# soedinglab/MMseqs2

Hardware: AMD Instinct MI355X
Metric: sw_gcells_per_s (higher is better)
Workload: dtype int16

## Files before the change

### mmseqs2_amd/csrc/pf_kernels.hip

```cpp
#include <type_traits>

#include "mmgpu_internal.h"
#include "pf_device.h"

namespace mmgpu {

namespace {

__device__ __forceinline__ PfCand *cand_slot(const PfDedupArgs &A, uint64_t bucket, uint32_t k) {
    return k < (uint32_t)PF_CAND0 ? A.cand_small + bucket * PF_CAND0 + k : A.cand + (A.cand_base[bucket] - A.cand_origin) + k;
}

struct __attribute__((packed, aligned(4))) U32Pair {
    uint32_t a, b;
};
struct __attribute__((packed, aligned(4))) U32Quad {
    uint32_t a, b, c, d;
};


constexpr uint32_t PF_COFS_KMERS = 12, PF_COFS_DWORDS = 4;

__global__ __launch_bounds__(256) void pf_cofs_kernel(const uint32_t *offsets, uint64_t table, uint32_t *cofs) {
    const uint64_t blk = (uint64_t)blockIdx.x * 256u + threadIdx.x;
// ... 536 lines not shown
    return o;
}
template <int NW>
__device__ __forceinline__ void load_cells(const uint8_t *p, uint32_t (&w)[NW]) {
    static_assert(NW == 4 || NW == 6, "16 or 24 bytes");
    const uintptr_t u = reinterpret_cast<uintptr_t>(p);
    const uint32_t *a = reinterpret_cast<const uint32_t *>(u & ~(uintptr_t)3);
    const uint32_t sh = (uint32_t)(u & 3u);
    const U32Quad d = *reinterpret_cast<const U32Quad *>(a);
    w[0] = __builtin_amdgcn_alignbyte(d.b, d.a, sh);
    w[1] = __builtin_amdgcn_alignbyte(d.c, d.b, sh);
    w[2] = __builtin_amdgcn_alignbyte(d.d, d.c, sh);
    if constexpr (NW == 4) {
        w[3] = __builtin_amdgcn_alignbyte(a[4], d.d, sh);
    } else {
        typedef uint32_t u32x3 __attribute__((ext_vector_type(3)));
        const u32x3 e = *reinterpret_cast<const u32x3 *>(a + 4);
        w[3] = __builtin_amdgcn_alignbyte(e.x, d.d, sh);
        w[4] = __builtin_amdgcn_alignbyte(e.y, e.x, sh);
        w[5] = __builtin_amdgcn_alignbyte(e.z, e.y, sh);
    }
}
template <int NW>
__device__ __forceinline__ Seg seg_cells_n(const uint32_t (&tw)[NW], const uint32_t (&qw)[NW], const uint32_t (&cw)[NW], int nn,
                                           const int8_t *smat) {
    Seg g;
    g.a = 0; g.b = 0; g.P = -(1 << 28); g.M = 0;
#pragma unroll
    for (int k = 0; k < 4 * NW; k++) {
        const uint32_t t5 = (tw[k >> 2] >> ((k & 3) * 8)) & 31u;
        const uint32_t q5 = (qw[k >> 2] >> ((k & 3) * 8)) & 31u;
        const int cb = (int)(int8_t)((cw[k >> 2] >> ((k & 3) * 8)) & 0xFFu);
        int x = (int)(int8_t)(smat[(q5 << 5) | t5] + cb);
        x = k < nn ? x : 0;
        g.b += x;
        g.a = max(0, g.a + x);
        g.P = max(g.P, g.b);
        g.M = max(g.M, g.a);
    }
    return g;
}
template <int NW>
__device__ __forceinline__ Seg seg_cells_rows_n(const uint32_t (&tw)[NW], const int8_t *rows, int nn) {
    Seg g;
    g.a = 0; g.b = 0; g.P = -(1 << 28); g.M = 0;
#pragma unroll
    for (int k = 0; k < 4 * NW; k++) {
        if (k < nn) {
            const int tb_ = (int)((tw[k >> 2] >> ((k & 3) * 8)) & 0xFFu);
            const int x = (int)rows[k * PF_PROW + (tb_ & (PF_PROW - 1))];
            g.b += x;
            g.a = max(0, g.a + x);
            g.P = max(g.P, g.b);
            g.M = max(g.M, g.a);
        }
    }
    return g;
}
__device__ __forceinline__ Seg seg_tree16(Seg g, int gl) {
#pragma unroll
    for (int d = 1; d < 16; d <<= 1) {
        Seg r;
        r.a = __shfl_down(g.a, d);
        r.b = __shfl_down(g.b, d);
        r.P = __shfl_down(g.P, d);
        r.M = __shfl_down(g.M, d);
        if ((gl & (2 * d - 1)) == 0) g = seg_combine(g, r);
    }
    return g;
}

template <bool SLOTS = true>
__device__ __forceinline__ uint64_t score_chunk(const PfDedupArgs &A, const int8_t *smat, uint64_t bucket, uint32_t q, uint32_t cb0,
                                                uint32_t nin, uint32_t ncand, PfCand c, int bshift, uint32_t *score_out = nullptr) {
    const int lane = lane_id();
    const int grp = lane >> 4, gl = lane & 15;
    const uint32_t qp0 = A.q_off[q];
    const int qlen = (int)(A.q_off[q + 1] - qp0);
    const uint8_t *qr = A.q_res + qp0;
    const uint8_t *qc = reinterpret_cast<const uint8_t *>(A.q_corr) + qp0;
    const bool has = (uint32_t)lane < nin;
    const int8_t *prows = (A.q_isprof && A.q_isprof[q]) ? A.q_rows + (size_t)qp0 * PF_PROW : nullptr;
    int my_len = 0, my_qs = 0;
    unsigned long long my_addr = 0;
    uint64_t cells = 0;
    if (has && !(A.q_nseg && A.q_nseg[q]))
        c.diag = (uint16_t)((c.diag & 0xFFu) | ((uint32_t)A.split_hi[(size_t)A.q_tile_base[q] * PF_T + c.score] << 8));
    if (has) {
        const int d = (int)(short)c.diag;
        const int tlen = (int)A.t_len[c.id];
        const uint8_t *t = A.t_res + (size_t)A.t_off4[c.id] * 4;
        const int mind = d < 0 ? -d : d;
        int ts = 0;
        if (d >= 0 && mind < qlen) {
            my_len = min(tlen, qlen - mind);
            my_qs = mind;
        } else if (d < 0 && mind < tlen) {
            my_len = min(tlen - mind, qlen);
            ts = mind;
        }
        my_addr = (unsigned long long)reinterpret_cast<uintptr_t>(t + ts);
        cells = (uint64_t)my_len;
        if (tlen >= 32768 && A.q_flags) atomicOr(&A.q_flags[q], 1u);
    }
    int my_score = 0;
    constexpr int UN = 2;
    auto trip = [&](auto nw_tag, const uint32_t k0) {
        constexpr int NW = decltype(nw_tag)::value;
        constexpr int CPL = 4 * NW, PASS = 16 * CPL;
        uint32_t tw[UN][NW], qw[UN][NW], cw[UN][NW];
        int len_u[UN], qs_u[UN];
        unsigned long long addr_u[UN];
#pragma unroll
        for (int u = 0; u < UN; u++) {
            const int src = (int)k0 + u * 4 + grp;
            len_u[u] = __shfl(my_len, src);
            qs_u[u] = __shfl(my_qs, src);
            addr_u[u] = __shfl(my_addr, src);
            if ((uint32_t)src >= nin) len_u[u] = 0;
#pragma unroll
            for (int z = 0; z < NW; z++) { tw[u][z] = 0; qw[u][z] = 0; cw[u][z] = 0; }
            if (gl * CPL < len_u[u]) {
                load_cells<NW>(reinterpret_cast<const uint8_t *>((uintptr_t)addr_u[u]) + gl * CPL, tw[u]);
                if (!prows) {
                    load_cells<NW>(qr + qs_u[u] + gl * CPL, qw[u]);
                    load_cells<NW>(qc + qs_u[u] + gl * CPL, cw[u]);
                }
            }
        }
#pragma unroll
        for (int u = 0; u < UN; u++) {
            const int len = len_u[u];
            Seg g;
            g.a = 0; g.b = 0; g.P = -(1 << 28); g.M = 0;
            if (gl * CPL < len) {
                if (prows) g = seg_cells_rows_n<NW>(tw[u], prows + (size_t)(qs_u[u] + gl * CPL) * PF_PROW, min(CPL, len - gl * CPL));
                else g = seg_cells_n<NW>(tw[u], qw[u], cw[u], min(CPL, len - gl * CPL), smat);
            }
            g = seg_tree16(g, gl);
            int sc = 0, best = 0;
            if (gl == 0 && len > 0) {
                best = max(g.M, g.P);
                sc = max(g.a, g.b);
            }
            int maxlen = len;
            maxlen = max(maxlen, __shfl_xor(maxlen, 16));
            maxlen = max(maxlen, __shfl_xor(maxlen, 32));
            for (int p0 = PASS; p0 < maxlen; p0 += PASS) {
                const int o = p0 + gl * CPL;
                Seg h;
                h.a = 0; h.b = 0; h.P = -(1 << 28); h.M = 0;
                if (o < len) {
                    uint32_t t2[NW], q2[NW], c2[NW];
                    load_cells<NW>(reinterpret_cast<const uint8_t *>((uintptr_t)addr_u[u]) + o, t2);
                    if (prows) h = seg_cells_rows_n<NW>(t2, prows + (size_t)(qs_u[u] + o) * PF_PROW, min(CPL, len - o));
                    else {
                        load_cells<NW>(qr + qs_u[u] + o, q2);
                        load_cells<NW>(qc + qs_u[u] + o, c2);
                        h = seg_cells_n<NW>(t2, q2, c2, min(CPL, len - o), smat);
                    }
                }
                h = seg_tree16(h, gl);
                if (gl == 0 && p0 < len) {
                    best = max(best, max(h.M, sc + h.P));
                    sc = max(h.a, sc + h.b);
                }
            }
            const int r0 = __shfl(best, 0), r1 = __shfl(best, 16), r2 = __shfl(best, 32), r3 = __shfl(best, 48);
            const int rel = lane - ((int)k0 + u * 4);
            if (rel >= 0 && rel < 4) my_score = rel == 0 ? r0 : (rel == 1 ? r1 : (rel == 2 ? r2 : r3));
        }
    };
    for (uint32_t k0 = 0; k0 < nin; k0 += 4 * UN) {
        const bool mine = (uint32_t)lane >= k0 && (uint32_t)lane < k0 + 4u * UN && has;
        if (ballot(mine && my_len > 256)) trip(std::integral_constant<int, 6>{}, k0);
        else trip(std::integral_constant<int, 4>{}, k0);
    }
    c.score = (uint32_t)my_score;
    if (score_out) *score_out = c.score;
    if constexpr (!SLOTS) return cells;
    if (has) {
        PfCand *slot = cand_slot(A, bucket, cb0 + (uint32_t)lane);
// ... 26 lines not shown
    return cells;
}

constexpr int REPLAY_WAVES_PER_EU = 4;
constexpr int REPLAY_PD = 4;


struct ReplayLds {
    uint32_t prev[4][PF_IDS_PER_BIN / 4];
    uint32_t last[4][PF_IDS_PER_BIN / 4];
    uint32_t emit[4][PF_IDS_PER_BIN / 32];
    uint32_t cand[4][3][64];
    uint8_t mark[4][64];
    int8_t smat[32 * 32];
};

__device__ __forceinline__ uint32_t lds_byte_exchange(uint32_t *word, uint32_t shift, uint32_t byte) {
    uint32_t old;
    const uint32_t addr = (uint32_t)(uintptr_t)word;
    asm volatile("ds_mskor_rtn_b32 %0, %1, %2, %3\n\ts_waitcnt lgkmcnt(0)" : "=v"(old) : "v"(addr), "v"(0xFFu << shift), "v"(byte << shift) : "memory");
    return old;
}

template <bool SEGS>
__device__ __forceinline__ void replay_bucket_impl(const PfDedupArgs &A, ReplayLds &M, uint64_t bucket) {
    const int lane = lane_id(), wave = (int)(threadIdx.x >> 6);
    const uint32_t B = A.bins;
    const uint32_t q = (uint32_t)(bucket / B), bin = (uint32_t)(bucket % B);
    const uint32_t ntiles = A.q_ntiles[q];
    if (ntiles == 0) {
        if (lane == 0) A.cand_count[bucket] = 0;
        return;
    }
    const uint32_t tb = A.q_tile_base[q];
    uint32_t *P = M.prev[wave];
    uint32_t *L = M.last[wave];
    uint32_t *E = M.emit[wave];
    uint8_t *mark = M.mark[wave];
    const int bshift = pf_bin_shift(B);
    auto clear_state = [&]() {
        uint4 *P4 = reinterpret_cast<uint4 *>(P);
        for (int k = lane; k < PF_IDS_PER_BIN / 16; k += 64) P4[k] = make_uint4(0u, 0u, 0u, 0u);
        for (int k = lane; k < PF_IDS_PER_BIN / 32; k += 64) E[k] = 0;
    };
    clear_state();

    uint32_t ncand = 0;
// ... 90 lines not shown
        request(64u, e1, tile1, at1);
        request(128u, e2, tile2, at2);
        request(192u, e3, tile3, at3);
        for (uint32_t xg = 0; xg < total; xg += 64u * REPLAY_PD) {
            one_round(xg, e0, tile0, at0);
            one_round(xg + 64u, e1, tile1, at1);
            one_round(xg + 128u, e2, tile2, at2);
            one_round(xg + 192u, e3, tile3, at3);
        }
    }
    if (lane == 0) {
        A.cand_count[bucket] = ncand;
        if (!SEGS && ncand > 64 && A.big_list) A.big_list[atomicAdd(A.big_count, 1u)] = (uint32_t)(bucket - (uint64_t)A.q_first * B);
    }
    if (!SEGS && ncand > 0 && ncand <= 64) {
        PfCand c = pf_cand_zero();
        if ((uint32_t)lane < ncand) {
            const uint32_t kd = M.cand[wave][0][lane];
            c.id = ((kd & 0xFFFu) << bshift) | bin;
            c.arr = M.cand[wave][1][lane];
            c.diag = (uint16_t)(kd >> 12);
            c.score = M.cand[wave][2][lane];
        }
        uint64_t cells = score_chunk(A, M.smat, bucket, q, 0, ncand, ncand, c, bshift);
        if (A.cell_counter) wave_sum_to((unsigned long long *)&A.cell_counter[q], cells);
    }
}

__global__ __launch_bounds__(256) __attribute__((amdgpu_waves_per_eu(REPLAY_WAVES_PER_EU))) void pf_replay_kernel(PfDedupArgs A) {
    __shared__ ReplayLds M;
    pf_load_smat32<256>(M.smat, A.mat, A.alphabet);
    __syncthreads();
    uint64_t bucket;
    if (!pf_wave_bucket(A, 4u, &bucket)) return;
    if (A.q_nseg && A.q_nseg[(uint32_t)(bucket / A.bins)]) replay_bucket_impl<true>(A, M, bucket);
    else replay_bucket_impl<false>(A, M, bucket);
}

__device__ __forceinline__ void ungapped_bucket(const PfDedupArgs &A, const int8_t *smat, uint64_t bucket) {
    const int lane = lane_id();
    const uint32_t B = A.bins;
    const uint32_t ncand = A.cand_count[bucket];
    const uint32_t q = (uint32_t)(bucket / B);
    if (ncand <= 64 || (A.q_nseg && A.q_nseg[q])) return;
    const int bshift = pf_bin_shift(B);
    uint64_t cells = 0;
    for (uint32_t cb0 = 0; cb0 < ncand; cb0 += 64) {
        const uint32_t nin = min(64u, ncand - cb0);
        PfCand c = pf_cand_zero();
        if ((uint32_t)lane < nin) c = *cand_slot(A, bucket, cb0 + (uint32_t)lane);
        cells += score_chunk(A, smat, bucket, q, cb0, nin, ncand, c, bshift);
    }
    if (A.cell_counter) wave_sum_to((unsigned long long *)&A.cell_counter[q], cells);
}

__global__ __launch_bounds__(256) void pf_ungapped_kernel(PfDedupArgs A) {
    __shared__ int8_t smat[32 * 32];
    const int wave = (int)(threadIdx.x >> 6);
    pf_load_smat32<256>(smat, A.mat, A.alphabet);
    __syncthreads();
    const uint32_t B = A.bins;
    if (A.big_list) {
        const uint32_t n = *A.big_count;
        for (uint32_t i = blockIdx.x * 4u + (uint32_t)wave; i < n; i += gridDim.x * 4u) ungapped_bucket(A, smat, (uint64_t)A.q_first * B + A.big_list[i]);
        return;
    }
    const uint64_t bucket = (uint64_t)A.q_first * B + (uint64_t)blockIdx.x * 4u + (uint32_t)wave;
    if (bucket >= (uint64_t)(A.q_first + A.n_queries) * B) return;
    ungapped_bucket(A, smat, bucket);
}

__global__ __launch_bounds__(256) void pf_count_kernel(PfDedupArgs A) {
    __shared__ uint16_t s_state[4][PF_IDS_PER_BIN];
    __shared__ uint32_t s_emit[4][PF_IDS_PER_BIN / 32];
    const int lane = lane_id(), wave = (int)(threadIdx.x >> 6);
    const uint32_t B = A.bins;
    uint64_t bucket;
    if (!pf_wave_bucket(A, 4u, &bucket)) return;
    const uint32_t q = (uint32_t)(bucket / B), bin = (uint32_t)(bucket % B);
    const uint32_t ntiles = A.q_ntiles[q];
    if (lane == 0) A.cand_count[bucket] = 0;
    if (ntiles == 0) return;
    const uint32_t tb = A.q_tile_base[q];
    uint16_t *S = s_state[wave];
    uint32_t *E = s_emit[wave];
    const int bshift = pf_bin_shift(B);
    for (int k = lane; k < PF_IDS_PER_BIN; k += 64) S[k] = 0;
    for (int k = lane; k < PF_IDS_PER_BIN / 32; k += 64) E[k] = 0;
    uint32_t ncand = 0;
    const uint64_t below = lanes_below(lane);
    for (uint32_t t0 = 0; t0 < ntiles; t0 += 64) {
        const uint32_t tl = t0 + (uint32_t)lane;
// ... 127 lines not shown
            const PfCand *cp = cand_slot(A, bucket, ci);
            atomicMax(&S[cp->id >> bshift], keepmax_key(min(255u, cp->score), ci));
        }
        __syncthreads();
        PfCand *surv = A.surv + (A.cand_base[(uint64_t)q * B] - A.cand_origin);
        for (uint32_t c0 = 0; c0 < ncand; c0 += 1024) {
            const uint32_t ci = c0 + threadIdx.x;
            bool win = false;
            PfCand c = pf_cand_zero();
            if (ci < ncand) {
                c = *cand_slot(A, bucket, ci);
                const uint32_t cnt = min(255u, c.score);
                win = S[c.id >> bshift] == keepmax_key(cnt, ci) && cnt >= A.min_diag_score;
            }
            wave_append(&A.surv_count[q], surv, win, c);
        }
        __syncthreads();
    }
}

constexpr int PF_LONG_POOL = 4096;
constexpr uint32_t PF_LONG_NONE = 0xFFFFu;

__device__ int wave_diag_score(const int8_t *smat, const uint8_t *qr, const uint8_t *qc, const int8_t *prows, int qlen, const uint8_t *t,
                               int tlen, int diag) {
    const int lane = lane_id();
    const int mind = diag < 0 ? -diag : diag;
    int len, qs, ts;
    if (diag >= 0 && mind < qlen) {
        len = min(tlen, qlen - mind);
        qs = mind;
        ts = 0;
    } else if (diag < 0 && mind < tlen) {
        len = min(tlen - mind, qlen);
        qs = 0;
        ts = mind;
    } else {
        return 0;
    }
    int sc = 0, best = 0;
    for (int p0 = 0; p0 < len; p0 += 1024) {
        const int o = p0 + lane * 16;
        Seg h;
        h.a = 0; h.b = 0; h.P = -(1 << 28); h.M = 0;
        if (o < len) {
            uint32_t tw[4], qw[4], cw[4];
            load_cells<4>(t + ts + o, tw);
            if (prows) h = seg_cells_rows_n<4>(tw, prows + (size_t)(qs + o) * PF_PROW, min(16, len - o));
            else {
                load_cells<4>(qr + qs + o, qw);
                load_cells<4>(qc + qs + o, cw);
                h = seg_cells_n<4>(tw, qw, cw, min(16, len - o), smat);
            }
        }
        h = seg_tree16(h, lane & 15);
        Seg g[4];
#pragma unroll
        for (int k = 0; k < 4; k++) {
            g[k].a = __shfl(h.a, 16 * k);
            g[k].b = __shfl(h.b, 16 * k);
            g[k].P = __shfl(h.P, 16 * k);
            g[k].M = __shfl(h.M, 16 * k);
        }
        const Seg all = seg_combine(seg_combine(g[0], g[1]), seg_combine(g[2], g[3]));
        best = max(best, max(all.M, sc + all.P));
        sc = max(all.a, sc + all.b);
    }
    return best;
}

__device__ int wave_long_score(const int8_t *smat, const uint8_t *qr, const uint8_t *qc, const int8_t *prows, int qlen, const uint8_t *t,
                               int tlen, uint32_t diag16) {
    int total = 0;
    for (uint32_t d = 1; d <= 1u + (uint32_t)tlen / 32768u; d++)
        total = max(total, wave_diag_score(smat, qr, qc, prows, qlen, t, tlen, (int)(0u - d * 65536u + diag16)));
    for (uint32_t d = 0; d <= (uint32_t)qlen / 65536u; d++)
        total = max(total, wave_diag_score(smat, qr, qc, prows, qlen, t, tlen, (int)(d * 65536u + diag16)));
    return total;
}

__global__ __launch_bounds__(256) void pf_longq_kernel(PfDedupArgs A) {
    __shared__ int8_t smat[32 * 32];
    const int lane = lane_id();
    pf_load_smat32<256>(smat, A.mat, A.alphabet);
    __syncthreads();
    const uint32_t B = A.bins;
    uint64_t bucket;
    if (!pf_wave_bucket(A, 4u, &bucket)) return;
    const uint32_t q = (uint32_t)(bucket / B);
    const uint32_t qp0 = A.q_off[q];
    const int qlen = (int)(A.q_off[q + 1] - qp0);
    if (qlen < 32768) return;
    if (lane == 0 && bucket == (uint64_t)q * B) atomicOr(&A.q_flags[q], 1u);
    if (A.nucl || (A.q_nseg && A.q_nseg[q])) return;
    const uint8_t *qr = A.q_res + qp0;
    const uint8_t *qc = reinterpret_cast<const uint8_t *>(A.q_corr) + qp0;
    const int8_t *prows = (A.q_isprof && A.q_isprof[q]) ? A.q_rows + (size_t)qp0 * PF_PROW : nullptr;
    const uint32_t ncand = A.cand_count[bucket];
    for (uint32_t ci = 0; ci < ncand; ci++) {
        PfCand *slot = cand_slot(A, bucket, ci);
        const uint32_t id = slot->id;
        const int own = wave_long_score(smat, qr, qc, prows, qlen, A.t_res + (size_t)A.t_off4[id] * 4, (int)A.t_len[id], slot->diag);
        if (lane == 0) slot->score = (uint32_t)own;
    }
}

__global__ __launch_bounds__(256) void pf_long_kernel(PfDedupArgs A) {
    __shared__ uint32_t s_tab[PF_IDS_PER_BIN];
    __shared__ uint32_t s_dbits[65536 / 32];
    __shared__ uint64_t s_key[PF_LONG_POOL];
    __shared__ uint32_t s_ci[PF_LONG_POOL];
    __shared__ uint16_t s_bucket[PF_LONG_POOL];
    __shared__ uint16_t s_job[PF_LONG_POOL];
    __shared__ int8_t smat[32 * 32];
    __shared__ uint32_t sh_npool, sh_nlong;
    const uint32_t q = A.q_first + blockIdx.x;
    if (!(A.q_flags[q] & 1u)) return;
    if (A.nucl || (A.q_nseg && A.q_nseg[q])) return;
    const int lane = lane_id(), wave = (int)(threadIdx.x >> 6);
    const uint32_t B = A.bins;
    const int bshift = pf_bin_shift(B);
    pf_load_smat32<256>(smat, A.mat, A.alphabet);
    for (int k = (int)threadIdx.x; k < 65536 / 32; k += 256) s_dbits[k] = 0;
    if (threadIdx.x == 0) {
        sh_npool = 0;
// ... 50 lines not shown
            uint32_t lo = p, hi = p;
            while (lo > 0 && (s_key[lo - 1] >> 43) == d) lo--;
            while (hi + 1 < npool && (s_key[hi + 1] >> 43) == d) hi++;
            const uint32_t r = p - lo, n_d = hi - lo + 1, b0 = (r / 8u) * 8u;
            if (b0 + 8u > n_d) job = (uint16_t)p;
            else {
                uint32_t h = 0;
                for (uint32_t z = lo + b0; z < p; z++) h += s_ci[z] >> 31;
                const uint32_t e = lo + b0 + h;
                job = (s_ci[e] >> 31) ? (uint16_t)e : (uint16_t)PF_LONG_NONE;
            }
            atomicAdd(&sh_nlong, 1u);
        }
        s_job[p] = job;
    }
    __syncthreads();
    const uint8_t *qr = A.q_res + qp0;
    const uint8_t *qc = reinterpret_cast<const uint8_t *>(A.q_corr) + qp0;
    const int8_t *prows = (A.q_isprof && A.q_isprof[q]) ? A.q_rows + (size_t)qp0 * PF_PROW : nullptr;
    for (uint32_t p = (uint32_t)wave; p < npool; p += 4) {
        if (!(s_ci[p] >> 31)) continue;
        PfCand *slot = cand_slot(A, (uint64_t)q * B + s_bucket[p], s_ci[p] & 0x7FFFFFFFu);
        const uint32_t id = slot->id, d16 = slot->diag;
        const int own = wave_long_score(smat, qr, qc, prows, qlen, A.t_res + (size_t)A.t_off4[id] * 4, (int)A.t_len[id], d16);
        int by = 0;
        const uint32_t job = s_job[p];
        if (job == p) by = own;
        else if (job != PF_LONG_NONE) {
            const uint32_t id2 = cand_slot(A, (uint64_t)q * B + s_bucket[job], s_ci[job] & 0x7FFFFFFFu)->id;
            by = wave_long_score(smat, qr, qc, prows, qlen, A.t_res + (size_t)A.t_off4[id2] * 4, (int)A.t_len[id2], d16);
        }
        const uint32_t cnt = (uint32_t)min(255, by), ex = (uint32_t)own;
        if (lane == 0) slot->score = (cnt == min(255u, ex)) ? ex : (0x80000000u | (cnt << 23) | (ex & 0x7FFFFFu));
    }
    }
    __threadfence();
    __syncthreads();
    if (threadIdx.x == 0) A.surv_count[q] = 0;
    __syncthreads();
    PfCand *surv = A.surv + (A.cand_base[(uint64_t)q * B] - A.cand_origin);
    for (uint32_t bk = 0; bk < B; bk++) {
        const uint64_t bucket = (uint64_t)q * B + bk;
        const uint32_t ncand = A.cand_count[bucket];
        if (ncand == 0) continue;
        for (uint32_t ci = threadIdx.x; ci < ncand; ci += 256) s_tab[cand_slot(A, bucket, ci)->id >> bshift] = 0;
        __syncthreads();
        for (uint32_t ci = threadIdx.x; ci < ncand; ci += 256) {
            const PfCand *cp = cand_slot(A, bucket, ci);
            atomicMax(&s_tab[cp->id >> bshift], keepmax_key(pf_el_count(cp->score), ci));
        }
        __syncthreads();
        for (uint32_t ci = threadIdx.x; ci < ncand; ci += 256) {
            const PfCand c = *cand_slot(A, bucket, ci);
// ... 105 lines not shown
        if (nseg >= (uint32_t)PF_MAX_SEG) { nseg = PF_MAX_SEG + 1; break; }
        nseg++;
        if (lane == 0) seg[nseg] = start;
        seg_begin = start;
        lcur = lo;
    }
    if (lane == 0) {
        A.q_nseg[q] = nseg;
        A.q_final[q] = total - seg_begin;
    }
}

__device__ __forceinline__ PfOvfElem ovf_from_cand(const PfCand &c, uint32_t step) {
    PfOvfElem e;
    e.id = c.id;
    e.score = 0;
    e.ord = ((long long)step << 33) + (long long)c.arr;
    e.diag = c.diag;
    e.pad0 = 0;
    e.pad1 = 0;
    return e;
}

__global__ __launch_bounds__(256) void pf_overflow_kernel(PfOvfArgs A) {
    __shared__ uint32_t s_tab[4][PF_IDS_PER_BIN];
    __shared__ int8_t smat[32 * 32];
    const PfDedupArgs &D = A.D;
    const int lane = lane_id(), wave = (int)(threadIdx.x >> 6);
    pf_load_smat32<256>(smat, D.mat, D.alphabet);
    __syncthreads();
    const uint32_t B = D.bins;
    const uint64_t w = (uint64_t)blockIdx.x * 4u + (uint32_t)wave;
    if (w >= (uint64_t)A.n_ovf * B) return;
    const uint32_t qi = (uint32_t)(w / B), bin = (uint32_t)(w % B);
    const uint32_t q = A.ovf_queries[qi];
    const uint32_t ns = D.q_nseg[q];
    const uint32_t step = A.step;
    if (ns > (uint32_t)PF_MAX_SEG || step > ns + 1) return;
    const bool final_step = step == ns + 1;
    if (final_step && A.q_final[q] == 0) return;
    const uint64_t bucket = (uint64_t)q * B + bin;
    const uint32_t ncand = D.cand_count[bucket];
    uint32_t *tab = s_tab[wave];
    const int bshift = pf_bin_shift(B);
    const uint64_t below = lanes_below(lane);
    const uint64_t base = A.ovf_base[qi] + (uint64_t)(D.cand_base[bucket] - D.cand_base[(uint64_t)q * B]);
// ... 93 lines not shown
        if (lane == 0) {
            A.o_count[(size_t)qi * B + bin] = n;
            if (n) atomicAdd(&totals[step], n);
        }
        return;
    }
    for (uint32_t r0 = 0; r0 < n; r0 += 64) {
        const uint32_t idx = r0 + (uint32_t)lane;
        const bool need = idx < n && cur[idx].score == 0;
        const uint64_t nb = ballot(need);
        if (!nb) continue;
        const uint32_t cnt = (uint32_t)__popcll(nb), mine = (uint32_t)__popcll(nb & below);
        if (need) tab[mine] = (uint32_t)lane;
        __builtin_amdgcn_wave_barrier();
        const int src = (uint32_t)lane < cnt ? (int)tab[lane] : 0;
        const uint32_t my_id = idx < n ? cur[idx].id : 0u, my_diag = idx < n ? (uint32_t)cur[idx].diag : 0u;
        PfCand c;
        c.id = (uint32_t)__shfl((int)my_id, src);
        c.arr = 0;
        c.score = 0;
        c.diag = (uint16_t)__shfl((int)my_diag, src);
        c.pad = 0;
        uint32_t sc = 0;
        (void)score_chunk<false>(D, smat, bucket, q, 0, cnt, 65u, c, bshift, &sc);
        tab[64 + lane] = sc;
        __builtin_amdgcn_wave_barrier();
        if (need) cur[idx].score = tab[64 + mine];
    }
    __threadfence();
    for (int k = lane; k < PF_IDS_PER_BIN; k += 64) tab[k] = 0;
    for (uint32_t r0 = 0; r0 < n; r0 += 64) {
        const uint32_t idx = r0 + (uint32_t)lane;
        if (idx < n) {
            const uint32_t cnt = min(255u, cur[idx].score);
            atomicMax(&tab[cur[idx].id >> bshift], keepmax_key(cnt, idx));
        }
    }
    PfOvfElem *dst = cur == O ? S : O;
    uint32_t m = 0;
    PfCand *surv = D.surv + (D.cand_base[(uint64_t)q * B] - D.cand_origin);
    for (uint32_t r0 = 0; r0 < n; r0 += 64) {
        const uint32_t idx = r0 + (uint32_t)lane;
        bool keep = false;
        PfOvfElem e;
        e.id = 0; e.score = 0; e.ord = 0; e.diag = 0; e.pad0 = 0; e.pad1 = 0;
        if (idx < n) {
            e = cur[idx];
// ... 37 lines not shown
            if (m) atomicAdd(&totals[step], m);
        }
    }
}

__device__ uint32_t list_ordinal(const PfSelectArgs &A, uint32_t q, uint32_t arr) {
    const uint32_t p0 = A.q_off[q], p1 = A.q_off[q + 1];
    uint32_t lo = p0, hi = p1 - 1;
    while (lo < hi) {
        const uint32_t mid = (lo + hi + 1) >> 1;
        if (A.peb[mid] <= arr) lo = mid; else hi = mid - 1;
    }
    const uint32_t rel = arr - A.peb[lo];
    uint32_t a = A.list_base[lo], b = A.list_base[lo + 1];
    if (b <= a) return a - A.list_base[p0];
    b -= 1;
    while (a < b) {
        const uint32_t mid = (a + b + 1) >> 1;
        if (A.lists[mid].lprefix <= rel) a = mid; else b = mid - 1;
    }
    return a - A.list_base[p0];
}

template <bool XCHG, bool BIG>
__global__ __launch_bounds__(256) void pf_select_kernel(PfSelectArgs A) {
    __shared__ uint32_t hist[256];
    __shared__ uint32_t sh_thr, sh_trunc, sh_nelig, sh_nsel, sh_ntie;
    __shared__ uint64_t sh_prefix, sh_mask;
    __shared__ uint32_t sh_remaining;
    __shared__ uint64_t skey_lds[BIG ? 1 : PF_MAX_HITS];
    __shared__ uint16_t sdiag_lds[BIG ? 1 : PF_MAX_HITS];
    const uint32_t q = A.q_first + blockIdx.x;
    uint64_t *skey = BIG ? A.big_keys + (size_t)q * A.big_stride : skey_lds;
    uint16_t *sdiag = BIG ? A.big_diags + (size_t)q * A.big_stride : sdiag_lds;
    const uint32_t sort_cap = BIG ? A.big_stride : (uint32_t)PF_MAX_HITS;
    const uint32_t n = A.surv_count[q];
    const PfCand *S = A.surv + (A.cand_base[(uint64_t)q * A.bins] - A.cand_origin);
    const uint32_t ident = A.q_identity[q];
    const uint32_t max_hits = A.max_hits;
    mmgpu_pf_hit *out = A.hits + (size_t)q * A.hit_stride;

    for (int k = (int)threadIdx.x; k < 256; k += 256) hist[k] = 0;
    if (threadIdx.x == 0) sh_remaining = 0;
    __syncthreads();
    if (A.cand_count != nullptr) {
        uint32_t loc = 0;
        for (uint32_t k = threadIdx.x; k < A.bins; k += 256) loc += A.cand_count[(uint64_t)q * A.bins + k];
        for (int d = 1; d < 64; d <<= 1) loc += __shfl_xor(loc, d);
        if ((threadIdx.x & 63u) == 0 && loc) atomicAdd(&sh_remaining, loc);
        __syncthreads();
        if (threadIdx.x == 0 && sh_remaining >= A.cand_cap && A.q_flags) A.q_flags[q] |= 2u;
        __syncthreads();
    }
    for (uint32_t k = threadIdx.x; k < n; k += 256) atomicAdd(&hist[pf_el_count(S[k].score)], 1u);
    __syncthreads();
    if (threadIdx.x == 0) {
        const uint32_t dthr = pf_score_threshold(hist, max_hits, A.min_diag_score);
        sh_thr = dthr;
        sh_trunc = (dthr >= 255u && !A.kmer_score) ? 1u : 0u;
        sh_nelig = 0;
        sh_nsel = 0;
    }
    __syncthreads();
    const uint32_t dthr = sh_thr;
    const bool trunc = sh_trunc != 0;
    const int ms = pf_self_clamp(A.q_self_score[q]);
    const float fms = (float)ms;
    const uint32_t refmask = A.ref_bins - 1;

    auto key_of = [&](const PfCand &c, bool *elig) -> uint64_t {
        const uint32_t cnt = pf_el_count(c.score);
        uint32_t kc;
        if (trunc) {
            *elig = cnt >= 255u && c.id != ident;
            kc = rescaled_count(pf_el_exact(c.score), fms);
        } else {
            *elig = cnt >= dthr && c.id != ident;
            kc = cnt;
        }
        const uint64_t ord = (A.nucl && cnt >= 255u) ? (uint64_t)c.id : (((uint64_t)c.pad << 32) | (uint64_t)c.arr);
        const uint32_t gid = XCHG ? A.global_ids[c.id] : c.id;
        if (XCHG) *elig = trunc ? cnt >= 255u : cnt >= dthr;
        return ((uint64_t)(255u - kc) << 56) | ((uint64_t)(gid & refmask) << 45) | (ord & ((1ull << 45) - 1));
    };

    uint32_t mine = 0;
    for (uint32_t k = threadIdx.x; k < n; k += 256) {
        bool el;
        (void)key_of(S[k], &el);
        mine += el ? 1u : 0u;
    }
    if (mine) atomicAdd(&sh_nelig, mine);
    __syncthreads();
    const uint32_t nelig = sh_nelig;
    const uint32_t has_ident = (!XCHG && ident != 0xFFFFFFFFu) ? 1u : 0u;
    const uint32_t want = max_hits > has_ident ? max_hits - has_ident : 0u;

    uint64_t kstar = ~0ull;
    if (nelig > want && want > 0) {
        if (threadIdx.x == 0) {
            sh_prefix = 0;
            sh_mask = 0;
            sh_remaining = want;
        }
        __syncthreads();
        for (int shift = 56; shift >= 0; shift -= 8) {
            for (int k = (int)threadIdx.x; k < 256; k += 256) hist[k] = 0;
            __syncthreads();
            const uint64_t prefix = sh_prefix, mask = sh_mask;
            for (uint32_t k = threadIdx.x; k < n; k += 256) {
                bool el;
                const uint64_t key = key_of(S[k], &el);
                if (el && (key & mask) == prefix) atomicAdd(&hist[(uint32_t)(key >> shift) & 0xFFu], 1u);
            }
            __syncthreads();
            if (threadIdx.x == 0) {
                uint32_t rem = sh_remaining, cum = 0, d = 0;
                for (d = 0; d < 256; d++) {
                    if (cum + hist[d] >= rem) break;
                    cum += hist[d];
                }
                sh_remaining = rem - cum;
                sh_prefix = prefix | ((uint64_t)d << shift);
                sh_mask = mask | (0xFFull << shift);
                sh_ntie = hist[d];
            }
            __syncthreads();
            if (!BIG && shift == 56 && sh_ntie <= sort_cap) {
                const uint32_t m = sh_ntie, rem = sh_remaining;
                const uint64_t prefix1 = sh_prefix;
                __syncthreads();
                if (threadIdx.x == 0) sh_ntie = 0;
                __syncthreads();
                for (uint32_t k = threadIdx.x; k < n; k += 256) {
                    bool el;
                    const uint64_t key = key_of(S[k], &el);
                    if (el && (key & (0xFFull << 56)) == prefix1) skey[atomicAdd(&sh_ntie, 1u)] = key;
                }
                uint32_t mp2 = 1;
                while (mp2 < m) mp2 <<= 1;
                __syncthreads();
                for (uint32_t k = m + threadIdx.x; k < mp2; k += 256) skey[k] = ~0ull;
                __syncthreads();
                block_bitonic_sort<256>(mp2, [&](uint32_t i, uint32_t j) { return skey[i] > skey[j]; }, [&](uint32_t i, uint32_t j) { exchange_at(skey, i, j); });
                if (threadIdx.x == 0) sh_prefix = skey[rem - 1];
                __syncthreads();
                break;
            }
        }
        kstar = sh_prefix;
// ... 170 lines not shown
    const uint64_t words = (table + 31) / 32;
    hipLaunchKernelGGL(pf_bitmap_kernel, dim3((unsigned)((words + 255) / 256)), dim3(256), 0, s, offsets, table, bitmap, nonempty);
    return hipGetLastError();
}

hipError_t launch_pf_scan(const uint32_t *in, const uint32_t *q_off, uint32_t nq, const uint64_t *base, uint32_t *out,
                          uint64_t *totals, hipStream_t s) {
    if (nq == 0) return hipSuccess;
    hipLaunchKernelGGL(pf_scan_kernel, dim3(nq), dim3(256), 0, s, in, q_off, nq, base, out, totals);
    return hipGetLastError();
}

hipError_t launch_pf_split(const PfSplitArgs &A, uint32_t n_tiles, hipStream_t s) {
    if (n_tiles == 0) return hipSuccess;
    hipLaunchKernelGGL(pf_split_kernel, dim3(n_tiles), dim3(SPW * 64), (size_t)SPW * A.bins * sizeof(uint16_t), s, A);
    return hipGetLastError();
}

hipError_t launch_pf_dedup(const PfDedupArgs &A, hipEvent_t after_replay, hipEvent_t after_ungapped, hipStream_t s) {
    const uint64_t buckets = (uint64_t)A.n_queries * A.bins;
    if (buckets == 0) return hipSuccess;
    const dim3 grid((unsigned)((buckets + 3) / 4)), block(256);
    hipError_t e;
    hipLaunchKernelGGL(pf_replay_kernel, grid, block, 0, s, A);
    if ((e = hipGetLastError()) != hipSuccess) return e;
    if (after_replay && (e = hipEventRecord(after_replay, s)) != hipSuccess) return e;
    const dim3 grid_big(A.big_list ? (unsigned)std::min<uint64_t>((buckets + 3) / 4, 2048) : grid.x);
    hipLaunchKernelGGL(pf_ungapped_kernel, grid_big, block, 0, s, A);
    if ((e = hipGetLastError()) != hipSuccess) return e;
    if (after_ungapped && (e = hipEventRecord(after_ungapped, s)) != hipSuccess) return e;
    if (A.nucl) hipLaunchKernelGGL(pf_keepmax_nucl_kernel, dim3((unsigned)((buckets + 1) / 2)), dim3(128), 0, s, A);
    else if (A.big_list) hipLaunchKernelGGL(pf_keepmax_list_kernel, dim3((unsigned)std::min<uint64_t>(buckets, 1024)), dim3(1024), 0, s, A);
    else hipLaunchKernelGGL(pf_keepmax_kernel, grid, block, 0, s, A);
    return hipGetLastError();
}

hipError_t launch_pf_long(const PfDedupArgs &A, bool long_queries, hipStream_t s) {
    if (A.n_queries == 0 || A.q_flags == nullptr) return hipSuccess;
    if (long_queries) {
        const uint64_t buckets = (uint64_t)A.n_queries * A.bins;
        hipLaunchKernelGGL(pf_longq_kernel, dim3((unsigned)((buckets + 3) / 4)), dim3(256), 0, s, A);
        if (hipError_t e = hipGetLastError(); e != hipSuccess) return e;
    }
    hipLaunchKernelGGL(pf_long_kernel, dim3(A.n_queries), dim3(256), 0, s, A);
    return hipGetLastError();
}

hipError_t launch_pf_count(const PfDedupArgs &A, hipEvent_t after_a, hipEvent_t after_b, hipStream_t s) {
    const uint64_t buckets = (uint64_t)A.n_queries * A.bins;
    if (buckets == 0) return hipSuccess;
    hipLaunchKernelGGL(pf_count_kernel, dim3((unsigned)((buckets + 3) / 4)), dim3(256), 0, s, A);
    hipError_t e = hipGetLastError();
    if (e != hipSuccess) return e;
    if (after_a && (e = hipEventRecord(after_a, s)) != hipSuccess) return e;
    if (after_b && (e = hipEventRecord(after_b, s)) != hipSuccess) return e;
    return hipSuccess;
}

hipError_t launch_pf_segments(const PfSegArgs &A, hipStream_t s) {
    if (A.n_ovf == 0) return hipSuccess;
    hipLaunchKernelGGL(pf_segments_kernel, dim3(A.n_ovf), dim3(64), 0, s, A);
    return hipGetLastError();
}

hipError_t launch_pf_overflow(const PfOvfArgs &A, hipStream_t s) {
    const uint64_t waves = (uint64_t)A.n_ovf * A.D.bins;
    if (waves == 0) return hipSuccess;
    hipLaunchKernelGGL(pf_overflow_kernel, dim3((unsigned)((waves + 3) / 4)), dim3(256), 0, s, A);
    return hipGetLastError();
}

hipError_t launch_pf_merge(const PfMergeArgs &A, hipStream_t s) {
    if (A.nq == 0) return hipSuccess;
    hipLaunchKernelGGL(pf_merge_kernel, dim3(A.nq), dim3(256), 0, s, A);
    return hipGetLastError();
}

hipError_t launch_pf_select(const PfSelectArgs &A, uint32_t nq, hipStream_t s) {
    if (nq == 0) return hipSuccess;
    if (A.xhits) hipLaunchKernelGGL((pf_select_kernel<true, false>), dim3(nq), dim3(256), 0, s, A);
    else if (A.big_keys) hipLaunchKernelGGL((pf_select_kernel<false, true>), dim3(nq), dim3(256), 0, s, A);
    else hipLaunchKernelGGL((pf_select_kernel<false, false>), dim3(nq), dim3(256), 0, s, A);
    return hipGetLastError();
}

void warm_pf() {
    hipFuncAttributes a;
    (void)hipFuncGetAttributes(&a, reinterpret_cast<const void *>(&pf_kmers_kernel<true>));
}

}
```

Measured before the change: 4899.

## Branch-free ungapped cells, DPP tree reduction, histogram-based eligibility and smaller select LDS

```diff
diff --git a/mmseqs2_amd/csrc/pf_kernels.hip b/mmseqs2_amd/csrc/pf_kernels.hip
--- a/mmseqs2_amd/csrc/pf_kernels.hip
+++ b/mmseqs2_amd/csrc/pf_kernels.hip
@@ -582,8 +582,8 @@
     }
 }
 template <int NW>
-__device__ __forceinline__ Seg seg_cells_n(const uint32_t (&tw)[NW], const uint32_t (&qw)[NW], const uint32_t (&cw)[NW], int nn,
-                                           const int8_t *smat) {
+__device__ __forceinline__ Seg seg_cells_select_n(const uint32_t (&tw)[NW], const uint32_t (&qw)[NW], const uint32_t (&cw)[NW], int nn,
+                                                  const int8_t *smat) {
     Seg g;
     g.a = 0; g.b = 0; g.P = -(1 << 28); g.M = 0;
 #pragma unroll
@@ -601,6 +601,37 @@
     return g;
 }
 template <int NW>
+__device__ __forceinline__ Seg seg_cells_n(const uint32_t (&tw)[NW], const uint32_t (&qw_in)[NW], const uint32_t (&cw_in)[NW], int nn,
+                                           const int8_t *smat, bool zrow) {
+    if (!zrow) return seg_cells_select_n<NW>(tw, qw_in, cw_in, nn, smat);
+    uint32_t qw[NW], cw[NW];
+#pragma unroll
+    for (int z = 0; z < NW; z++) { qw[z] = qw_in[z]; cw[z] = cw_in[z]; }
+    if (nn < 4 * NW) {
+#pragma unroll
+        for (int z = 0; z < NW; z++) {
+            const int bits = min(32, max(0, 8 * nn - 32 * z));
+            const uint32_t kill = (uint32_t)(0xFFFFFFFFull << bits);
+            qw[z] = (qw[z] & ~kill) | (0x1F1F1F1Fu & kill);
+            cw[z] &= ~kill;
+        }
+    }
+    Seg g;
+    g.a = 0; g.b = 0; g.P = -(1 << 28); g.M = 0;
+#pragma unroll
+    for (int k = 0; k < 4 * NW; k++) {
+        const uint32_t t5 = (tw[k >> 2] >> ((k & 3) * 8)) & 31u;
+        const uint32_t q5 = (qw[k >> 2] >> ((k & 3) * 8)) & 31u;
+        const int cb = (int)(int8_t)((cw[k >> 2] >> ((k & 3) * 8)) & 0xFFu);
+        const int x = (int)(int8_t)(smat[(q5 << 5) | t5] + cb);
+        g.b += x;
+        g.a = max(0, g.a + x);
+        g.P = max(g.P, g.b);
+        g.M = max(g.M, g.a);
+    }
+    return g;
+}
+template <int NW>
 __device__ __forceinline__ Seg seg_cells_rows_n(const uint32_t (&tw)[NW], const int8_t *rows, int nn) {
     Seg g;
     g.a = 0; g.b = 0; g.P = -(1 << 28); g.M = 0;
@@ -617,29 +648,38 @@
     }
     return g;
 }
+template <int D>
+__device__ __forceinline__ int row_shl(int v) { return __builtin_amdgcn_update_dpp(0, v, 0x100 + D , 0xF, 0xF, true); }
+template <int D>
+__device__ __forceinline__ Seg seg_tree_level(Seg g, int gl) {
+    Seg r;
+    r.a = row_shl<D>(g.a);
+    r.b = row_shl<D>(g.b);
+    r.P = row_shl<D>(g.P);
+    r.M = row_shl<D>(g.M);
+    if ((gl & (2 * D - 1)) == 0) g = seg_combine(g, r);
+    return g;
+}
 __device__ __forceinline__ Seg seg_tree16(Seg g, int gl) {
-#pragma unroll
-    for (int d = 1; d < 16; d <<= 1) {
-        Seg r;
-        r.a = __shfl_down(g.a, d);
-        r.b = __shfl_down(g.b, d);
-        r.P = __shfl_down(g.P, d);
-        r.M = __shfl_down(g.M, d);
-        if ((gl & (2 * d - 1)) == 0) g = seg_combine(g, r);
-    }
+    g = seg_tree_level<1>(g, gl);
+    g = seg_tree_level<2>(g, gl);
+    g = seg_tree_level<4>(g, gl);
+    g = seg_tree_level<8>(g, gl);
     return g;
 }
 
-template <bool SLOTS = true>
+template <bool ZROW, bool SLOTS = true>
 __device__ __forceinline__ uint64_t score_chunk(const PfDedupArgs &A, const int8_t *smat, uint64_t bucket, uint32_t q, uint32_t cb0,
                                                 uint32_t nin, uint32_t ncand, PfCand c, int bshift, uint32_t *score_out = nullptr) {
     const int lane = lane_id();
     const int grp = lane >> 4, gl = lane & 15;
+    bucket = ((uint64_t)__builtin_amdgcn_readfirstlane((uint32_t)(bucket >> 32)) << 32) | (uint64_t)__builtin_amdgcn_readfirstlane((uint32_t)bucket);
     const uint32_t qp0 = A.q_off[q];
     const int qlen = (int)(A.q_off[q + 1] - qp0);
     const uint8_t *qr = A.q_res + qp0;
     const uint8_t *qc = reinterpret_cast<const uint8_t *>(A.q_corr) + qp0;
     const bool has = (uint32_t)lane < nin;
+    constexpr bool zrow = ZROW;
     const int8_t *prows = (A.q_isprof && A.q_isprof[q]) ? A.q_rows + (size_t)qp0 * PF_PROW : nullptr;
     int my_len = 0, my_qs = 0;
     unsigned long long my_addr = 0;
@@ -660,7 +700,7 @@
             ts = mind;
         }
         my_addr = (unsigned long long)reinterpret_cast<uintptr_t>(t + ts);
-        cells = (uint64_t)my_len;
+        cells = (uint64_t)(uint32_t)my_len;
         if (tlen >= 32768 && A.q_flags) atomicOr(&A.q_flags[q], 1u);
     }
     int my_score = 0;
@@ -695,7 +735,7 @@
             g.a = 0; g.b = 0; g.P = -(1 << 28); g.M = 0;
             if (gl * CPL < len) {
                 if (prows) g = seg_cells_rows_n<NW>(tw[u], prows + (size_t)(qs_u[u] + gl * CPL) * PF_PROW, min(CPL, len - gl * CPL));
-                else g = seg_cells_n<NW>(tw[u], qw[u], cw[u], min(CPL, len - gl * CPL), smat);
+                else g = seg_cells_n<NW>(tw[u], qw[u], cw[u], min(CPL, len - gl * CPL), smat, zrow);
             }
             g = seg_tree16(g, gl);
             int sc = 0, best = 0;
@@ -717,7 +757,7 @@
                     else {
                         load_cells<NW>(qr + qs_u[u] + o, q2);
                         load_cells<NW>(qc + qs_u[u] + o, c2);
-                        h = seg_cells_n<NW>(t2, q2, c2, min(CPL, len - o), smat);
+                        h = seg_cells_n<NW>(t2, q2, c2, min(CPL, len - o), smat, zrow);
                     }
                 }
                 h = seg_tree16(h, gl);
@@ -790,7 +830,7 @@
     return old;
 }
 
-template <bool SEGS>
+template <bool SEGS, bool ZROW>
 __device__ __forceinline__ void replay_bucket_impl(const PfDedupArgs &A, ReplayLds &M, uint64_t bucket) {
     const int lane = lane_id(), wave = (int)(threadIdx.x >> 6);
     const uint32_t B = A.bins;
@@ -927,21 +967,23 @@
             c.diag = (uint16_t)(kd >> 12);
             c.score = M.cand[wave][2][lane];
         }
-        uint64_t cells = score_chunk(A, M.smat, bucket, q, 0, ncand, ncand, c, bshift);
+        uint64_t cells = score_chunk<ZROW>(A, M.smat, bucket, q, 0, ncand, ncand, c, bshift);
         if (A.cell_counter) wave_sum_to((unsigned long long *)&A.cell_counter[q], cells);
     }
 }
 
+template <bool ZROW>
 __global__ __launch_bounds__(256) __attribute__((amdgpu_waves_per_eu(REPLAY_WAVES_PER_EU))) void pf_replay_kernel(PfDedupArgs A) {
     __shared__ ReplayLds M;
     pf_load_smat32<256>(M.smat, A.mat, A.alphabet);
     __syncthreads();
     uint64_t bucket;
     if (!pf_wave_bucket(A, 4u, &bucket)) return;
-    if (A.q_nseg && A.q_nseg[(uint32_t)(bucket / A.bins)]) replay_bucket_impl<true>(A, M, bucket);
-    else replay_bucket_impl<false>(A, M, bucket);
-}
-
+    if (A.q_nseg && A.q_nseg[(uint32_t)(bucket / A.bins)]) replay_bucket_impl<true, ZROW>(A, M, bucket);
+    else replay_bucket_impl<false, ZROW>(A, M, bucket);
+}
+
+template <bool ZROW>
 __device__ __forceinline__ void ungapped_bucket(const PfDedupArgs &A, const int8_t *smat, uint64_t bucket) {
     const int lane = lane_id();
     const uint32_t B = A.bins;
@@ -954,11 +996,12 @@
         const uint32_t nin = min(64u, ncand - cb0);
         PfCand c = pf_cand_zero();
         if ((uint32_t)lane < nin) c = *cand_slot(A, bucket, cb0 + (uint32_t)lane);
-        cells += score_chunk(A, smat, bucket, q, cb0, nin, ncand, c, bshift);
+        cells += score_chunk<ZROW>(A, smat, bucket, q, cb0, nin, ncand, c, bshift);
     }
     if (A.cell_counter) wave_sum_to((unsigned long long *)&A.cell_counter[q], cells);
 }
 
+template <bool ZROW>
 __global__ __launch_bounds__(256) void pf_ungapped_kernel(PfDedupArgs A) {
     __shared__ int8_t smat[32 * 32];
     const int wave = (int)(threadIdx.x >> 6);
@@ -967,12 +1010,12 @@
     const uint32_t B = A.bins;
     if (A.big_list) {
         const uint32_t n = *A.big_count;
-        for (uint32_t i = blockIdx.x * 4u + (uint32_t)wave; i < n; i += gridDim.x * 4u) ungapped_bucket(A, smat, (uint64_t)A.q_first * B + A.big_list[i]);
+        for (uint32_t i = blockIdx.x * 4u + (uint32_t)wave; i < n; i += gridDim.x * 4u) ungapped_bucket<ZROW>(A, smat, (uint64_t)A.q_first * B + A.big_list[i]);
         return;
     }
     const uint64_t bucket = (uint64_t)A.q_first * B + (uint64_t)blockIdx.x * 4u + (uint32_t)wave;
     if (bucket >= (uint64_t)(A.q_first + A.n_queries) * B) return;
-    ungapped_bucket(A, smat, bucket);
+    ungapped_bucket<ZROW>(A, smat, bucket);
 }
 
 __global__ __launch_bounds__(256) void pf_count_kernel(PfDedupArgs A) {
@@ -1146,7 +1189,7 @@
 constexpr int PF_LONG_POOL = 4096;
 constexpr uint32_t PF_LONG_NONE = 0xFFFFu;
 
-__device__ int wave_diag_score(const int8_t *smat, const uint8_t *qr, const uint8_t *qc, const int8_t *prows, int qlen, const uint8_t *t,
+__device__ int wave_diag_score(const int8_t *smat, bool zrow, const uint8_t *qr, const uint8_t *qc, const int8_t *prows, int qlen, const uint8_t *t,
                                int tlen, int diag) {
     const int lane = lane_id();
     const int mind = diag < 0 ? -diag : diag;
@@ -1174,7 +1217,7 @@
             else {
                 load_cells<4>(qr + qs + o, qw);
                 load_cells<4>(qc + qs + o, cw);
-                h = seg_cells_n<4>(tw, qw, cw, min(16, len - o), smat);
+                h = seg_cells_n<4>(tw, qw, cw, min(16, len - o), smat, zrow);
             }
         }
         h = seg_tree16(h, lane & 15);
@@ -1193,13 +1236,13 @@
     return best;
 }
 
-__device__ int wave_long_score(const int8_t *smat, const uint8_t *qr, const uint8_t *qc, const int8_t *prows, int qlen, const uint8_t *t,
+__device__ int wave_long_score(const int8_t *smat, bool zrow, const uint8_t *qr, const uint8_t *qc, const int8_t *prows, int qlen, const uint8_t *t,
                                int tlen, uint32_t diag16) {
     int total = 0;
     for (uint32_t d = 1; d <= 1u + (uint32_t)tlen / 32768u; d++)
-        total = max(total, wave_diag_score(smat, qr, qc, prows, qlen, t, tlen, (int)(0u - d * 65536u + diag16)));
+        total = max(total, wave_diag_score(smat, zrow, qr, qc, prows, qlen, t, tlen, (int)(0u - d * 65536u + diag16)));
     for (uint32_t d = 0; d <= (uint32_t)qlen / 65536u; d++)
-        total = max(total, wave_diag_score(smat, qr, qc, prows, qlen, t, tlen, (int)(d * 65536u + diag16)));
+        total = max(total, wave_diag_score(smat, zrow, qr, qc, prows, qlen, t, tlen, (int)(d * 65536u + diag16)));
     return total;
 }
 
@@ -1224,7 +1267,7 @@
     for (uint32_t ci = 0; ci < ncand; ci++) {
         PfCand *slot = cand_slot(A, bucket, ci);
         const uint32_t id = slot->id;
-        const int own = wave_long_score(smat, qr, qc, prows, qlen, A.t_res + (size_t)A.t_off4[id] * 4, (int)A.t_len[id], slot->diag);
+        const int own = wave_long_score(smat, A.alphabet <= 31, qr, qc, prows, qlen, A.t_res + (size_t)A.t_off4[id] * 4, (int)A.t_len[id], slot->diag);
         if (lane == 0) slot->score = (uint32_t)own;
     }
 }
@@ -1321,13 +1364,13 @@
         if (!(s_ci[p] >> 31)) continue;
         PfCand *slot = cand_slot(A, (uint64_t)q * B + s_bucket[p], s_ci[p] & 0x7FFFFFFFu);
         const uint32_t id = slot->id, d16 = slot->diag;
-        const int own = wave_long_score(smat, qr, qc, prows, qlen, A.t_res + (size_t)A.t_off4[id] * 4, (int)A.t_len[id], d16);
+        const int own = wave_long_score(smat, A.alphabet <= 31, qr, qc, prows, qlen, A.t_res + (size_t)A.t_off4[id] * 4, (int)A.t_len[id], d16);
         int by = 0;
         const uint32_t job = s_job[p];
         if (job == p) by = own;
         else if (job != PF_LONG_NONE) {
             const uint32_t id2 = cand_slot(A, (uint64_t)q * B + s_bucket[job], s_ci[job] & 0x7FFFFFFFu)->id;
-            by = wave_long_score(smat, qr, qc, prows, qlen, A.t_res + (size_t)A.t_off4[id2] * 4, (int)A.t_len[id2], d16);
+            by = wave_long_score(smat, A.alphabet <= 31, qr, qc, prows, qlen, A.t_res + (size_t)A.t_off4[id2] * 4, (int)A.t_len[id2], d16);
         }
         const uint32_t cnt = (uint32_t)min(255, by), ex = (uint32_t)own;
         if (lane == 0) slot->score = (cnt == min(255u, ex)) ? ex : (0x80000000u | (cnt << 23) | (ex & 0x7FFFFFu));
@@ -1479,6 +1522,7 @@
     return e;
 }
 
+template <bool ZROW>
 __global__ __launch_bounds__(256) void pf_overflow_kernel(PfOvfArgs A) {
     __shared__ uint32_t s_tab[4][PF_IDS_PER_BIN];
     __shared__ int8_t smat[32 * 32];
@@ -1618,7 +1662,7 @@
         c.diag = (uint16_t)__shfl((int)my_diag, src);
         c.pad = 0;
         uint32_t sc = 0;
-        (void)score_chunk<false>(D, smat, bucket, q, 0, cnt, 65u, c, bshift, &sc);
+        (void)score_chunk<ZROW, false>(D, smat, bucket, q, 0, cnt, 65u, c, bshift, &sc);
         tab[64 + lane] = sc;
         __builtin_amdgcn_wave_barrier();
         if (need) cur[idx].score = tab[64 + mine];
@@ -1702,18 +1746,19 @@
     return a - A.list_base[p0];
 }
 
-template <bool XCHG, bool BIG>
+constexpr int PF_SELECT_SMALL = 512;
+template <bool XCHG, bool BIG, int CAP>
 __global__ __launch_bounds__(256) void pf_select_kernel(PfSelectArgs A) {
     __shared__ uint32_t hist[256];
-    __shared__ uint32_t sh_thr, sh_trunc, sh_nelig, sh_nsel, sh_ntie;
+    __shared__ uint32_t sh_thr, sh_trunc, sh_nelig, sh_nsel, sh_ntie, sh_ident_cls;
     __shared__ uint64_t sh_prefix, sh_mask;
     __shared__ uint32_t sh_remaining;
-    __shared__ uint64_t skey_lds[BIG ? 1 : PF_MAX_HITS];
-    __shared__ uint16_t sdiag_lds[BIG ? 1 : PF_MAX_HITS];
+    __shared__ uint64_t skey_lds[BIG ? 1 : CAP];
+    __shared__ uint16_t sdiag_lds[BIG ? 1 : CAP];
     const uint32_t q = A.q_first + blockIdx.x;
     uint64_t *skey = BIG ? A.big_keys + (size_t)q * A.big_stride : skey_lds;
     uint16_t *sdiag = BIG ? A.big_diags + (size_t)q * A.big_stride : sdiag_lds;
-    const uint32_t sort_cap = BIG ? A.big_stride : (uint32_t)PF_MAX_HITS;
+    const uint32_t sort_cap = BIG ? A.big_stride : (uint32_t)CAP;
     const uint32_t n = A.surv_count[q];
     const PfCand *S = A.surv + (A.cand_base[(uint64_t)q * A.bins] - A.cand_origin);
     const uint32_t ident = A.q_identity[q];
@@ -1721,7 +1766,13 @@
     mmgpu_pf_hit *out = A.hits + (size_t)q * A.hit_stride;
 
     for (int k = (int)threadIdx.x; k < 256; k += 256) hist[k] = 0;
-    if (threadIdx.x == 0) sh_remaining = 0;
+    constexpr uint32_t NO_CLASS = 0xFFFFFFFFu;
+    if (threadIdx.x == 0) {
+        sh_remaining = 0;
+        sh_ident_cls = NO_CLASS;
+        sh_nelig = 0;
+        sh_nsel = 0;
+    }
     __syncthreads();
     if (A.cand_count != nullptr) {
         uint32_t loc = 0;
@@ -1732,14 +1783,17 @@
         if (threadIdx.x == 0 && sh_remaining >= A.cand_cap && A.q_flags) A.q_flags[q] |= 2u;
         __syncthreads();
     }
-    for (uint32_t k = threadIdx.x; k < n; k += 256) atomicAdd(&hist[pf_el_count(S[k].score)], 1u);
+    for (uint32_t k = threadIdx.x; k < n; k += 256) {
+        const PfCand c = S[k];
+        const uint32_t cnt = pf_el_count(c.score);
+        atomicAdd(&hist[cnt], 1u);
+        if (!XCHG && c.id == ident) sh_ident_cls = cnt;
+    }
     __syncthreads();
     if (threadIdx.x == 0) {
         const uint32_t dthr = pf_score_threshold(hist, max_hits, A.min_diag_score);
         sh_thr = dthr;
         sh_trunc = (dthr >= 255u && !A.kmer_score) ? 1u : 0u;
-        sh_nelig = 0;
-        sh_nsel = 0;
     }
     __syncthreads();
     const uint32_t dthr = sh_thr;
@@ -1764,13 +1818,13 @@
         return ((uint64_t)(255u - kc) << 56) | ((uint64_t)(gid & refmask) << 45) | (ord & ((1ull << 45) - 1));
     };
 
-    uint32_t mine = 0;
-    for (uint32_t k = threadIdx.x; k < n; k += 256) {
-        bool el;
-        (void)key_of(S[k], &el);
-        mine += el ? 1u : 0u;
-    }
-    if (mine) atomicAdd(&sh_nelig, mine);
+    const uint32_t cut = trunc ? 255u : dthr;
+    const uint32_t ident_cls = sh_ident_cls;
+    {
+        uint32_t mine = threadIdx.x >= cut ? hist[threadIdx.x] - (threadIdx.x == ident_cls ? 1u : 0u) : 0u;
+        for (int d = 1; d < 64; d <<= 1) mine += __shfl_xor(mine, d);
+        if ((threadIdx.x & 63u) == 0 && mine) atomicAdd(&sh_nelig, mine);
+    }
     __syncthreads();
     const uint32_t nelig = sh_nelig;
     const uint32_t has_ident = (!XCHG && ident != 0xFFFFFFFFu) ? 1u : 0u;
@@ -1785,6 +1839,21 @@
         }
         __syncthreads();
         for (int shift = 56; shift >= 0; shift -= 8) {
+            if (shift == 56 && !trunc) {
+                if (threadIdx.x == 0) {
+                    uint32_t rem = want, cum = 0, cls = 255, h = 0;
+                    for (;; cls--) {
+                        h = hist[cls] - (cls == ident_cls ? 1u : 0u);
+                        if (cum + h >= rem || cls == cut) break;
+                        cum += h;
+                    }
+                    sh_remaining = rem - cum;
+                    sh_prefix = (uint64_t)(255u - cls) << 56;
+                    sh_mask = 0xFFull << 56;
+                    sh_ntie = h;
+                }
+                __syncthreads();
+            } else {
             for (int k = (int)threadIdx.x; k < 256; k += 256) hist[k] = 0;
             __syncthreads();
             const uint64_t prefix = sh_prefix, mask = sh_mask;
@@ -1806,6 +1875,7 @@
                 sh_ntie = hist[d];
             }
             __syncthreads();
+            }
             if (!BIG && shift == 56 && sh_ntie <= sort_cap) {
                 const uint32_t m = sh_ntie, rem = sh_remaining;
                 const uint64_t prefix1 = sh_prefix;
@@ -2022,11 +2092,14 @@
     if (buckets == 0) return hipSuccess;
     const dim3 grid((unsigned)((buckets + 3) / 4)), block(256);
     hipError_t e;
-    hipLaunchKernelGGL(pf_replay_kernel, grid, block, 0, s, A);
+    const bool zrow = A.alphabet <= 31;
+    if (zrow) hipLaunchKernelGGL(pf_replay_kernel<true>, grid, block, 0, s, A);
+    else hipLaunchKernelGGL(pf_replay_kernel<false>, grid, block, 0, s, A);
     if ((e = hipGetLastError()) != hipSuccess) return e;
     if (after_replay && (e = hipEventRecord(after_replay, s)) != hipSuccess) return e;
     const dim3 grid_big(A.big_list ? (unsigned)std::min<uint64_t>((buckets + 3) / 4, 2048) : grid.x);
-    hipLaunchKernelGGL(pf_ungapped_kernel, grid_big, block, 0, s, A);
+    if (zrow) hipLaunchKernelGGL(pf_ungapped_kernel<true>, grid_big, block, 0, s, A);
+    else hipLaunchKernelGGL(pf_ungapped_kernel<false>, grid_big, block, 0, s, A);
     if ((e = hipGetLastError()) != hipSuccess) return e;
     if (after_ungapped && (e = hipEventRecord(after_ungapped, s)) != hipSuccess) return e;
     if (A.nucl) hipLaunchKernelGGL(pf_keepmax_nucl_kernel, dim3((unsigned)((buckets + 1) / 2)), dim3(128), 0, s, A);
@@ -2066,7 +2139,8 @@
 hipError_t launch_pf_overflow(const PfOvfArgs &A, hipStream_t s) {
     const uint64_t waves = (uint64_t)A.n_ovf * A.D.bins;
     if (waves == 0) return hipSuccess;
-    hipLaunchKernelGGL(pf_overflow_kernel, dim3((unsigned)((waves + 3) / 4)), dim3(256), 0, s, A);
+    if (A.D.alphabet <= 31) hipLaunchKernelGGL(pf_overflow_kernel<true>, dim3((unsigned)((waves + 3) / 4)), dim3(256), 0, s, A);
+    else hipLaunchKernelGGL(pf_overflow_kernel<false>, dim3((unsigned)((waves + 3) / 4)), dim3(256), 0, s, A);
     return hipGetLastError();
 }
 
@@ -2078,9 +2152,10 @@
 
 hipError_t launch_pf_select(const PfSelectArgs &A, uint32_t nq, hipStream_t s) {
     if (nq == 0) return hipSuccess;
-    if (A.xhits) hipLaunchKernelGGL((pf_select_kernel<true, false>), dim3(nq), dim3(256), 0, s, A);
-    else if (A.big_keys) hipLaunchKernelGGL((pf_select_kernel<false, true>), dim3(nq), dim3(256), 0, s, A);
-    else hipLaunchKernelGGL((pf_select_kernel<false, false>), dim3(nq), dim3(256), 0, s, A);
+    if (A.xhits) hipLaunchKernelGGL((pf_select_kernel<true, false, PF_MAX_HITS>), dim3(nq), dim3(256), 0, s, A);
+    else if (A.big_keys) hipLaunchKernelGGL((pf_select_kernel<false, true, PF_MAX_HITS>), dim3(nq), dim3(256), 0, s, A);
+    else if (A.max_hits <= (uint32_t)PF_SELECT_SMALL) hipLaunchKernelGGL((pf_select_kernel<false, false, PF_SELECT_SMALL>), dim3(nq), dim3(256), 0, s, A);
+    else hipLaunchKernelGGL((pf_select_kernel<false, false, PF_MAX_HITS>), dim3(nq), dim3(256), 0, s, A);
     return hipGetLastError();
 }
 
```

After: 4903 (median of 3 runs). About the same (+0.1%).
